# alexj94/future_urban_scene_generation

Hardware: AMD Instinct MI355X
Metric: synthesised vehicle crops/sec @256x256 (higher is better)
Workload: dtype f32 tensors; conv contraction as 3 fp16 MFMA products of scaled (hi, lo) operand splits, f32 accumulate (error vs fp64 <= 1.3x the exact-f32 MFMA kernel's: observed 0.96-1.27x over 12 operand scales x 5 layers; range-guarded; exact-f32 leg in precision_legs)

## Files before the change

### future_urban_scene_generation_amd/_lib.py

```python
from __future__ import annotations

import ctypes as C
import os

_HERE = os.path.dirname(os.path.abspath(__file__))
LIB_PATH = os.environ.get("FUSG_LIB", os.path.join(_HERE, "libfusg.so"))


class FusgUnavailable(RuntimeError):
    pass


class FusgError(RuntimeError):
    pass


class Tensor(C.Structure):
    _fields_ = [("data", C.c_void_p),
                ("n", C.c_int64), ("c", C.c_int64), ("h", C.c_int64), ("w", C.c_int64),
                ("sn", C.c_int64), ("sc", C.c_int64), ("sh", C.c_int64), ("sw", C.c_int64),
                ("dtype", C.c_int32), ("_pad", C.c_int32)]


class ConvDesc(C.Structure):
# ... 5 lines not shown
                ("stride", C.c_int32), ("upsample", C.c_int32), ("pad_mode", C.c_int32), ("pre_op", C.c_int32),
                ("act", C.c_int32), ("store_mode", C.c_int32), ("qh", C.c_int32), ("qw", C.c_int32),
                ("nphase", C.c_int32), ("out_sy", C.c_int32), ("out_sx", C.c_int32),
                ("out_oy", C.c_int32 * 4), ("out_ox", C.c_int32 * 4),
                ("dst_c_off", C.c_int32), ("tile", C.c_int32), ("ksplit", C.c_int32), ("precision", C.c_int32),
                ("wpack_h", C.c_void_p),
                ("kh", C.c_int32), ("kw", C.c_int32), ("dil", C.c_int32), ("pad_h", C.c_int32), ("pad_w", C.c_int32),
                ("wfrag_order", C.c_int32), ("wfrag", C.c_void_p), ("stats_out", C.c_void_p),
                ("tile_list", C.c_void_p), ("tile_count", C.c_int32), ("q_oy", C.c_int32), ("q_ox", C.c_int32),
                ("stats_slots", C.c_int32),
                ("wscale", C.c_void_p), ("status", C.c_void_p), ("wfrag_bf16", C.c_void_p), ("wfrag_f32", C.c_void_p),
                ("splitk_counters", C.c_void_p), ("splitk_counters_len", C.c_int32), ("tap_sparse", C.c_int32)]


class BneckDesc(C.Structure):
    _fields_ = [("x", Tensor), ("res", Tensor), ("dst", Tensor),
                ("pre_scale", C.c_void_p), ("pre_shift", C.c_void_p),
                ("w1frag", C.c_void_p), ("bias1", C.c_void_p), ("wscale1", C.c_void_p),
                ("w2frag", C.c_void_p), ("bias2", C.c_void_p), ("wscale2", C.c_void_p),
                ("w3frag", C.c_void_p), ("bias3", C.c_void_p), ("wscale3", C.c_void_p),
                ("status", C.c_void_p), ("planes", C.c_int32), ("exact_f32", C.c_int32)]


class PackSpec(C.Structure):
    _fields_ = [(n, C.c_int32) for n in ("cout", "cin", "kh", "kw", "c0", "stride", "pad", "dil", "upsample", "cin_pad")]


class PackSizes(C.Structure):
    _fields_ = [("cout_pad", C.c_int32), ("k_pad", C.c_int32), ("c0k", C.c_int32), ("c1k", C.c_int32),
                ("wfrag_order", C.c_int32), ("_pad", C.c_int32), ("wpack_floats", C.c_int64), ("ktab_ints", C.c_int64),
                ("wpack_h_halves", C.c_int64), ("wfrag_halves", C.c_int64)]


F32, U8, I32 = 0, 1, 2
PAD_ZERO, PAD_REFLECT, PAD_REPLICATE = 0, 1, 2
PRE_NONE, PRE_RELU, PRE_ELU, PRE_AFFINE_RELU, PRE_AFFINE = 0, 1, 2, 3, 4
ACT_NONE, ACT_RELU, ACT_TANH, ACT_SIGMOID, ACT_TANH01 = 0, 1, 2, 3, 4
STORE_NORMAL, STORE_D2S, STORE_S2D = 0, 1, 2
PREC_F32, PREC_F16X3, PREC_EMU_BF16, PREC_EMU_BF16X2, PREC_BF16 = 0, 1, 2, 3, 4
MAX_FRAMES = 64
TILE_AUTO, TILE_128x128, TILE_128x64, TILE_128x32, TILE_64x64, TILE_64x128 = 0, 1, 2, 3, 4, 5

_TP = C.POINTER(Tensor)
_SIGS = {
    "fusg_conv2d": (C.c_int, [C.POINTER(ConvDesc), C.c_void_p]),
    "fusg_conv2d_plan": (C.c_int64, [C.POINTER(ConvDesc)]),
    "fusg_conv2d_route": (C.c_int, [C.POINTER(ConvDesc)]),
    "fusg_hg_bottleneck": (C.c_int, [C.POINTER(BneckDesc), C.c_void_p]),
    "fusg_chan_stats": (C.c_int, [_TP, C.c_void_p, C.c_int32, C.c_void_p]),
    "fusg_in_finalize": (C.c_int, [_TP, C.c_void_p, C.c_int32, C.c_float, C.c_void_p, C.c_void_p, C.c_void_p]),
    "fusg_ln_finalize": (C.c_int, [_TP, C.c_void_p, C.c_int32, C.c_float, C.c_void_p, C.c_void_p, C.c_void_p,
                                   C.c_void_p, C.c_void_p]),
    "fusg_in_finalize_slots": (C.c_int, [C.c_void_p, C.c_int32, C.c_int32, C.c_int32, C.c_float, C.c_void_p, C.c_void_p, C.c_void_p]),
    "fusg_ln_finalize_slots": (C.c_int, [C.c_void_p, C.c_int32, C.c_int32, C.c_int32, C.c_float, C.c_void_p, C.c_void_p,
                                         C.c_void_p, C.c_void_p, C.c_void_p]),
    "fusg_affine_act": (C.c_int, [_TP, C.c_void_p, C.c_void_p, C.c_int64, C.c_int32, _TP, _TP, C.c_void_p]),
    "fusg_maxpool2": (C.c_int, [_TP, _TP, C.c_void_p]),
    "fusg_upsample2_add": (C.c_int, [_TP, _TP, _TP, C.c_void_p]),
    "fusg_copy4d": (C.c_int, [_TP, _TP, C.c_int32, C.c_void_p]),
    "fusg_add4d": (C.c_int, [_TP, _TP, _TP, C.c_void_p]),
    "fusg_space_to_depth2": (C.c_int, [_TP, _TP, C.c_void_p]),
    "fusg_depth_to_space2": (C.c_int, [_TP, _TP, C.c_void_p]),
    "fusg_ec_inputs": (C.c_int, [_TP, _TP, _TP, _TP, C.c_int32, C.c_void_p]),
    "fusg_hshift_sum": (C.c_int, [_TP, C.c_void_p, C.c_int32, C.c_int32, C.c_int32, C.c_int32, _TP, C.c_void_p]),
    "fusg_argmax_hw": (C.c_int, [_TP, C.c_void_p, C.c_void_p]),
    "fusg_to_image_u8": (C.c_int, [_TP, _TP, C.c_void_p]),
    "fusg_merge_u8": (C.c_int, [_TP, _TP, _TP, _TP, C.c_void_p]),
    "fusg_warp_perspective_u8": (C.c_int, [_TP, C.c_void_p, _TP, C.c_void_p]),
    "fusg_warp_perspective_indexed_u8": (C.c_int, [_TP, C.c_void_p, C.c_void_p, C.c_int32, _TP, C.c_void_p]),
    "fusg_warp_perspective_frames_u8": (C.c_int, [_TP, C.c_void_p, C.c_void_p, C.c_int32, C.c_int32, _TP, C.c_void_p]),
    "fusg_fill_poly_planes_u8": (C.c_int, [_TP, C.c_void_p, C.c_void_p, C.c_int32, _TP, C.c_void_p]),
# ... 34 lines not shown
    "fusg_plan_destroy": (None, [C.c_void_p]),
    "fusg_plan_begin": (C.c_int, [C.c_void_p]),
    "fusg_plan_end": (C.c_int, [C.c_void_p]),
    "fusg_plan_add_dependency": (C.c_int, [C.c_void_p, C.c_void_p, C.c_void_p]),
    "fusg_plan_add_h2d": (C.c_int, [C.c_void_p, C.c_void_p, C.c_void_p, C.c_int64, C.c_int32, C.c_int64, C.c_void_p]),
    "fusg_plan_next_slot": (C.c_int, [C.c_void_p]),
    "fusg_plan_size": (C.c_int64, [C.c_void_p]),
    "fusg_plan_run": (C.c_int, [C.c_void_p]),
    "fusg_plan_streams": (C.c_int32, [C.c_void_p]),
    "fusg_plan_run_mt": (C.c_int, [C.c_void_p]),
    "fusg_plan_graph_capture": (C.c_int, [C.c_void_p, C.c_void_p, C.c_int32]),
    "fusg_plan_graph_nodes": (C.c_int64, [C.c_void_p]),
    "fusg_plan_graph_slot": (C.c_int, [C.c_void_p]),
    "fusg_plan_graph_launch": (C.c_int, [C.c_void_p, C.c_void_p]),
    "fusg_pack_conv_sizes": (C.c_int, [C.POINTER(PackSpec), C.POINTER(PackSizes)]),
    "fusg_pack_conv_weights": (C.c_int, [C.POINTER(PackSpec)] + [C.c_void_p] * 8),
    "fusg_version": (C.c_int, []),
    "fusg_last_error": (C.c_char_p, []),
    "fusg_last_conv_kernel": (C.c_int, []),
    "fusg_arch": (C.c_char_p, []),
    "fusg_sizeof_tensor": (C.c_int, []),
    "fusg_sizeof_conv_desc": (C.c_int, []),
    "fusg_sizeof_bneck_desc": (C.c_int, []),
    "fusg_prof_enable": (None, [C.c_int]),
    "fusg_prof_reset": (None, []),
    "fusg_prof_read": (C.c_int, [C.c_int, C.POINTER(C.c_double), C.POINTER(C.c_int64), C.POINTER(C.c_double)]),
}
EXPORTS = tuple(_SIGS.keys())

_lib = None


def lib():
    global _lib
    if _lib is None:
        if not os.path.exists(LIB_PATH):
            raise FusgUnavailable(
                f"{LIB_PATH} not found: build it with `python -c 'import __graft_entry__ as g; g.build()'` "
                "(hipcc --offload-arch=gfx950).  There is no CPU fallback.")
        import torch
        try:
            h = C.CDLL(LIB_PATH)
        except OSError as e:
            raise FusgUnavailable(f"cannot load {LIB_PATH}: {e}") from e
        for name, (res, args) in _SIGS.items():
            fn = getattr(h, name)
            fn.restype = res
            fn.argtypes = args
        if (h.fusg_sizeof_tensor() != C.sizeof(Tensor) or h.fusg_sizeof_conv_desc() != C.sizeof(ConvDesc)
                or h.fusg_sizeof_bneck_desc() != C.sizeof(BneckDesc)):
            raise FusgUnavailable("libfusg.so struct layout differs from the ctypes mirror (stale build?)")
        _lib = h
    return _lib


def check(rc: int, what: str = "") -> None:
    if rc != 0:
        msg = lib().fusg_last_error()
        raise FusgError(f"{what}: rc={rc}: {msg.decode() if msg else ''}")
```

### future_urban_scene_generation_amd/csrc/common.h

```cpp
#pragma once
#include <hip/hip_runtime.h>
#include <functional>
#include <memory>
#include <tuple>
#include <utility>
#include <stdint.h>
#include <stdio.h>
#include <string.h>
#include "../../include/fusg.h"

namespace fusg {

void set_error(const char* fmt, ...);
void note_conv_kernel(int kind);

#define FUSG_CHECK(cond, ...)                         \
    do {                                              \
        if (!(cond)) {                                \
            fusg::set_error(__VA_ARGS__);             \
            return FUSG_ERR_INVALID;                  \
        }                                             \
    } while (0)

#define FUSG_LAUNCH_CHECK(what)                                                    \
// ... 32 lines not shown

template <class A> struct SavedArg {
    A a;
    explicit SavedArg(A v) : a(v) {}
    A get() const { return a; }
};
template <> struct SavedArg<const fusg_tensor*> {
    bool has; fusg_tensor t;
    explicit SavedArg(const fusg_tensor* p) : has(p != nullptr), t(p ? *p : fusg_tensor{}) {}
    const fusg_tensor* get() const { return has ? &t : nullptr; }
};
template <> struct SavedArg<const fusg_conv_desc*> {
    bool has; fusg_conv_desc d;
    explicit SavedArg(const fusg_conv_desc* p) : has(p != nullptr), d(p ? *p : fusg_conv_desc{}) {}
    const fusg_conv_desc* get() const { return has ? &d : nullptr; }
};

template <> struct SavedArg<const fusg_bneck_desc*> {
    bool has; fusg_bneck_desc d;
    explicit SavedArg(const fusg_bneck_desc* p) : has(p != nullptr), d(p ? *p : fusg_bneck_desc{}) {}
    const fusg_bneck_desc* get() const { return has ? &d : nullptr; }
};

template <class... A>
int plan_dispatch(int (*impl)(A..., void*), void* stream, A... a) {
    if (plan_recording()) {
        auto saved = std::make_shared<std::tuple<SavedArg<A>...>>(SavedArg<A>(a)...);
        plan_append((hipStream_t)stream, [impl, saved](hipStream_t s) {
            return std::apply([&](const SavedArg<A>&... sv) { return impl(sv.get()..., (void*)s); }, *saved);
        });
    }
    return impl(a..., stream);
}

const float* zero_line();

void prof_begin(int kind, hipStream_t s, double flops);
void prof_end(int kind, hipStream_t s);

}
```

### future_urban_scene_generation_amd/ops.py

```python
from __future__ import annotations

import ctypes as C
from typing import Optional, Tuple

import torch

from . import _lib as L
from .pack import ConvPlan

_DT = {torch.float32: L.F32, torch.uint8: L.U8, torch.int32: L.I32}

import os as _os
import numpy as _np


def _env_set(name: str) -> bool:
    return name in _os.environ


_PREC = {"f32": L.PREC_F32, "f16x3": L.PREC_F16X3,
         "bf16": L.PREC_BF16,
         "emu_bf16": L.PREC_EMU_BF16, "emu_bf16x2": L.PREC_EMU_BF16X2}
_EMU_BITS = {"emu_bf16": 8, "emu_bf16x2": 16}

# ... 444 lines not shown
    d.pre_scale, d.pre_shift = p["pre"][0].data_ptr(), p["pre"][1].data_ptr()
    if RECORDER is not None:
        RECORDER.keep.append(p["pre"])
    for i, key in ((1, "c1"), (2, "c2"), (3, "c3")):
        plan = p[key].to(x.device)
        dev = plan.dev
        if RECORDER is not None:
            RECORDER.keep.append(dev)
        assert dev.get("wfrag") is not None and dev["wfrag_order"] == 0, key
        frag = plan.frag_f32_dev() if f32 else dev["wfrag"]
        assert frag is not None, key
        if RECORDER is not None:
            RECORDER.keep.append(frag)
        setattr(d, "w%dfrag" % i, frag.data_ptr())
        setattr(d, "bias%d" % i, dev["bias"].data_ptr())
        setattr(d, "wscale%d" % i, dev["wscale"].data_ptr())
    d.status = status_word(x.device).data_ptr()
    d.planes = planes
    d.exact_f32 = 1 if f32 else 0
    L.check(L.lib().fusg_hg_bottleneck(C.byref(d), stream_ptr()), "hg_bottleneck")
    return out


def last_conv_kernel() -> int:
    return int(L.lib().fusg_last_conv_kernel())


_BORDER_TILES = {}


def border_tiles(h: int, w: int, device) -> torch.Tensor:
    key = (h, w, str(device))
    t = _BORDER_TILES.get(key)
    if t is None:
        ny, nx = h // 8, w // 16
        idx = [y * nx + x for y in range(ny) for x in range(nx) if y in (0, ny - 1) or x in (0, nx - 1)]
        t = torch.tensor(idx, dtype=torch.int32, device=device)
        _BORDER_TILES[key] = t
    return t


def up2_phases_ok(x: torch.Tensor, precision: Optional[str] = None) -> bool:
    b, c, h, w = x.shape
    return h >= 2 and w >= 2 and _os.environ.get("FUSG_NO_UP2_PHASES") is None


# ... 431 lines not shown
```

### future_urban_scene_generation_amd/vunet/models.py

```python
from __future__ import annotations

import argparse
from typing import List, Optional, Sequence

import torch
import torch.nn as nn

from .. import _lib as L
from .. import ops, pack
from ..nn_base import FusedNet, WNConvP, WNConvTP, entry_point
from .layers import (Activation, DeConv2d, DepthToSpace, DownSample, MyConv2d, NiN, Residual, Sampler, SpaceToDepth,
                     UpSample)


def _res(c_in, c_out, dp, wn):
    return Residual(c_in=c_in, c_out=c_out, activation=Activation("elu"), drop_prob=dp, w_norm=wn)


class AutoRegressiveBlock(nn.Module):
    def __init__(self, drop_prob, w_norm):
        super().__init__()
        self.s2d = SpaceToDepth(2)
        self.d2s = DepthToSpace(2)
        self.residual_init = _res(256, 128, drop_prob, w_norm)
# ... 145 lines not shown
            if name == "shape_decoder_6.conv" and w.shape[0] * w.shape[3] <= 32 and split is None and m.stride == 1:
                P[name] = pack.pack_conv_rowsplit(w, h.bias, pad=m.padding).to(device)
                continue
            P[name] = pack.pack_conv(w, h.bias, c_split=split, stride=m.stride, pad=m.padding).to(device)
        return P

    def _residual(self, name: str, x, skip=None, out=None):
        return ops.conv(self._plans[name + ".layers.2"], x, skip, pre_op=L.PRE_ELU, res0=x, out=out)

    def _nin(self, name: str, x, x1=None, out=None):
        return ops.conv(self._plans[name + ".layers.1"], x, x1, pre_op=L.PRE_ELU, out=out)

    _UP_PLAN = {"subpixel": ".depth4x", "conv2d_t": ".up", "nearest": ".conv"}

    def _upsample(self, name: str, x):
        return ops.conv(self._plans[name + self._UP_PLAN[self.up_mode]], x, store=L.STORE_D2S)

    @staticmethod
    def _subbatch(b: int) -> int:
        import os
        n = int(os.environ.get("FUSG_VU_SUBBATCH", "0"))
        return n if 0 < n < b else 0

    def _shape_encoder_top(self, x, n):
        b, _, h, w = x.shape
        dev = x.device
        sb, sc = ops.nhwc_empty(b, 32, h, w, dev), ops.nhwc_empty(b, 32, h, w, dev)
        ab, ac = ops.nhwc_empty(b, 32, h // 2, w // 2, dev), ops.nhwc_empty(b, 32, h // 2, w // 2, dev)
        a1 = ops.nhwc_empty(b, 32, h // 2, w // 2, dev)
        for lo in range(0, b, n):
            hi = min(b, lo + n)
            t = self._nin("shape_encoder_1.nin", x[lo:hi])
            s0 = self._residual("shape_encoder_1.residual_0", t)
            s1 = self._residual("shape_encoder_1.residual_1", s0)
            self._nin("shape_skip_1_b", s0, out=sb[lo:hi])
            self._nin("shape_skip_1_c", s1, out=sc[lo:hi])
            d = ops.conv(self._plans["shape_encoder_1_a.down.down"], s1)
            a0 = self._residual("shape_encoder_1_a.residual_0", d)
            self._residual("shape_encoder_1_a.residual_1", a0, out=a1[lo:hi])
            self._nin("shape_skip_1_a_b", a0, out=ab[lo:hi])
            self._nin("shape_skip_1_a_c", a1[lo:hi], out=ac[lo:hi])
        return a1, [sb, sc, ab, ac]

    def _shape_decoder_tail(self, x, skips, n):
        b, _, h, w = x.shape
        head = self._plans["shape_decoder_6.conv"]
        out = torch.empty((b, 3, 2 * h, 2 * w), device=x.device, dtype=torch.float32)
        for lo in range(0, b, n):
            hi = min(b, lo + n)
            r = self._residual("shape_decoder_5_a.residual_0", x[lo:hi], skips[0][lo:hi])
            r = self._residual("shape_decoder_5_a.residual_1", r, skips[1][lo:hi])
            u = self._upsample("shape_decoder_5_a.up", r)
            e = self._residual("shape_decoder_6.residual_0", u, skips[2][lo:hi])
            e = self._residual("shape_decoder_6.residual_1", e, skips[3][lo:hi])
            o = ops.conv_rowsplit(head, e, nchw_out=True) if head.rowsplit is not None else ops.conv(head, e, nchw_out=True)
            ops.copy4d(o, out[lo:hi], 0)
        return out

    def set_vehicle_seeds(self, seeds=None):
        if seeds is None:
            self.__dict__.pop("_vehicle_gens", None)
            return
        gens = []
        for sd in seeds:
            g = torch.Generator(device="cpu")
            g.manual_seed(int(sd))
# ... 58 lines not shown
    def _sampler(self, name: str, x, noise, mu_out=None, c_off=0, z_out=None):
        p = self._plans[name + ".conv"]
        if mu_out is None:
            mu = ops.conv(p, x)
        else:
            ops.conv(p, x, out=mu_out, out_c_off=c_off)
            mu = mu_out[:, c_off:c_off + p.cout]
        assert tuple(noise.shape) == tuple(mu.shape), (noise.shape, mu.shape)
        z = ops.add4d(mu, noise, None if z_out is None else z_out[:, c_off:c_off + p.cout])
        return mu, z

    def _init_block(self, name, x):
        x = self._nin(name + ".nin", x)
        s0 = x = self._residual(name + ".residual_0", x)
        s1 = x = self._residual(name + ".residual_1", x)
        return x, [s0, s1]

    def _down_block(self, name, x):
        x = ops.conv(self._plans[name + ".down.down"], x)
        s0 = x = self._residual(name + ".residual_0", x)
        s1 = x = self._residual(name + ".residual_1", x)
        return x, [s0, s1]

    def _up_block(self, name, x, skip_a, skip_b):
        x = self._residual(name + ".residual_0", x, skip_a)
        x = self._residual(name + ".residual_1", x, skip_b)
        return self._upsample(name + ".up", x)

    def _ar_block(self, name, x, skip_a, enc_down_mu, noise):
        x = self._residual(name + ".residual_init", x, skip_a)
        x_ = ops.space_to_depth2(self._residual(name + ".residual_s2d", x))
        g = None
        if enc_down_mu is not None:
            gs = ops.space_to_depth2(ops.as_nhwc(enc_down_mu))
            g = [self._nin(f"{name}.nin_{k}", gs[:, 128 * k:128 * (k + 1)]) for k in range(3)]
        b, _, h, w = x_.shape
        mus = ops.nhwc_empty(b, 512, h, w, x_.device)
        zs = ops.nhwc_empty(b, 512, h, w, x_.device)
        for k in range(4):
            _, z_k = self._sampler(f"{name}.sampler_{k}", x_, noise[k], mus, 128 * k, zs)
            if k < 3:
                cond = g[k] if g is not None else self._nin(f"{name}.nin_{k}", z_k)
                x_ = self._residual(f"{name}.residual_{k}", x_, cond)
        return x, ops.depth_to_space2(mus), ops.depth_to_space2(zs)

    @entry_point
    def forward_enc_up(self, x):
        self._ensure(x)
        x = ops.as_nhwc(x)
        x, _ = self._init_block("app_encoder_1", x)
        names = ["app_encoder_1_a", "app_encoder_1_b"] + (["app_encoder_1_c"] if self.vunet_256 else []) + \
                ["app_encoder_2", "app_encoder_3"]
        for n in names:
            x, _ = self._down_block(n, x)
        skips = [self._nin("app_skip_3_c", x)]
        x, sl = self._down_block("app_encoder_4", x)
        outputs = [sl[-2], x]
        skips.append(self._nin("app_skip_4_c", x))
        return outputs, skips

    @entry_point
    def forward_dec_up(self, x):
        self._ensure(x)
        x = ops.as_nhwc(x)
        skips: List[torch.Tensor] = []
        nsub = self._subbatch(x.shape[0]) if self.vunet_256 else 0
        if nsub:
            x, skips = self._shape_encoder_top(x, nsub)
        else:
            x, sl = self._init_block("shape_encoder_1", x)
            skips += [self._nin("shape_skip_1_b", sl[-2]), self._nin("shape_skip_1_c", sl[-1])]
            if self.vunet_256:
                x, sl = self._down_block("shape_encoder_1_a", x)
                skips += [self._nin("shape_skip_1_a_b", sl[-2]), self._nin("shape_skip_1_a_c", sl[-1])]
        for i in range(2, 7):
            x, sl = self._down_block(f"shape_encoder_{i}", x)
            skips += [self._nin(f"shape_skip_{i}_b", sl[-2]), self._nin(f"shape_skip_{i}_c", sl[-1])]
        return [x], skips

    @entry_point
    def forward_enc_down(self, enc_up_outputs: Sequence[torch.Tensor], skips: Sequence[torch.Tensor]):
        self._ensure(enc_up_outputs[-1])
        P = self._plans
        o1, o2 = ops.as_nhwc(enc_up_outputs[-1]), ops.as_nhwc(enc_up_outputs[-2])
        b, _, h, w = o1.shape
        noise = self._draw_noise([(b, 128, h, w), (b, 128, 2 * h, 2 * w)], o1.device)
        x = ops.conv(P["app_bottleneck"], o1)
        x = self._residual("app_decoder_1_a", x, ops.as_nhwc(skips[-1]))
        mu_0, z_0 = self._sampler("app_decoder_1_b", x, noise[0])
        x_ = ops.conv(P["app_decoder_1_c"], o2, z_0)
        x = self._residual("app_decoder_1_d", x, x_)
        x = self._upsample("app_decoder_1_e", x)
        x = self._residual("app_decoder_2_a", x, None)
        mu_1, z_1 = self._sampler("app_decoder_2_b", x, noise[1])
        return [mu_0, mu_1], [z_0, z_1]

    @entry_point
# ... 55 lines not shown
```

### include/fusg.h

```cpp
#ifndef FUSG_H
#define FUSG_H

#include <stdint.h>

#ifdef __cplusplus
extern "C" {
#endif

#define FUSG_VERSION 118

typedef enum fusg_status {
    FUSG_OK = 0,
    FUSG_ERR_INVALID = -1,
    FUSG_ERR_LAUNCH = -2,
    FUSG_ERR_UNSUPPORTED = -3
} fusg_status;

typedef enum fusg_dtype { FUSG_F32 = 0, FUSG_U8 = 1, FUSG_I32 = 2 } fusg_dtype;

typedef struct fusg_tensor {
    void*   data;
    int64_t n, c, h, w;
    int64_t sn, sc, sh, sw;
    int32_t dtype;
// ... 77 lines not shown
    const void*    wfrag_f32;
    int32_t*       splitk_counters;
    int32_t        splitk_counters_len;
    int32_t        tap_sparse;
} fusg_conv_desc;

int  fusg_conv2d(const fusg_conv_desc* d, void* stream);
int64_t fusg_conv2d_plan(fusg_conv_desc* d);
int  fusg_conv2d_route(const fusg_conv_desc* d);

typedef struct fusg_bneck_desc {
    fusg_tensor x, res, dst;
    const float* pre_scale;
    const float* pre_shift;
    const void*  w1frag; const float* bias1; const float* wscale1;
    const void*  w2frag; const float* bias2; const float* wscale2;
    const void*  w3frag; const float* bias3; const float* wscale3;
    int32_t*     status;
    int32_t      planes;
    int32_t      exact_f32;
} fusg_bneck_desc;
int fusg_hg_bottleneck(const fusg_bneck_desc* d, void* stream);

typedef struct fusg_pack_spec {
    int32_t cout, cin, kh, kw;
    int32_t c0;
    int32_t stride, pad, dil;
    int32_t upsample;
    int32_t cin_pad;
} fusg_pack_spec;
typedef struct fusg_pack_sizes {
    int32_t cout_pad, k_pad, c0k, c1k;
    int32_t wfrag_order;
    int32_t _pad;
    int64_t wpack_floats;
    int64_t ktab_ints;
    int64_t wpack_h_halves;
    int64_t wfrag_halves;
} fusg_pack_sizes;
int fusg_pack_conv_sizes(const fusg_pack_spec* spec, fusg_pack_sizes* sizes);
int fusg_pack_conv_weights(const fusg_pack_spec* spec, const float* weight, const float* bias, float* wpack, int32_t* ktab,
                           float* bias_pad, uint16_t* wpack_h, float* wscale, uint16_t* wfrag);


int fusg_chan_stats(const fusg_tensor* x, float* partial, int32_t nchunk, void* stream);
int fusg_in_finalize(const fusg_tensor* x, const float* partial, int32_t nchunk, float eps,
// ... 127 lines not shown
int        fusg_plan_begin(fusg_plan* p);
int        fusg_plan_end(fusg_plan* p);
int        fusg_plan_add_dependency(fusg_plan* p, void* waiter, void* signaller);
int        fusg_plan_add_h2d(fusg_plan* p, void* dst, const void* src, int64_t bytes, int32_t nslots, int64_t slot_stride, void* stream);
int        fusg_plan_next_slot(fusg_plan* p);
int64_t    fusg_plan_size(const fusg_plan* p);
int        fusg_plan_run(fusg_plan* p);
int32_t    fusg_plan_streams(fusg_plan* p);
int        fusg_plan_run_mt(fusg_plan* p);
int        fusg_plan_graph_capture(fusg_plan* p, void* capture_stream, int32_t slot);
int64_t    fusg_plan_graph_nodes(const fusg_plan* p);
int        fusg_plan_graph_slot(fusg_plan* p);
int        fusg_plan_graph_launch(fusg_plan* p, void* stream);


int         fusg_version(void);
const char* fusg_last_error(void);
enum { FUSG_CONV_GENERIC_F32 = 0, FUSG_CONV_GENERIC_F16X3 = 1, FUSG_CONV_HALO = 2, FUSG_CONV_HALO_S2D = 3,
       FUSG_CONV_TAPUNIT = 4, FUSG_CONV_HALO_BF16 = 5, FUSG_CONV_BNECK = 6 ,
       FUSG_CONV_POINTWISE = 7 ,
       FUSG_CONV_SMALL = 8 ,
       FUSG_CONV_HALO_F32 = 9 ,
       FUSG_CONV_TAPUNIT_F32 = 10 ,
       FUSG_CONV_TAPUNIT_BF16 = 11  };
int         fusg_last_conv_kernel(void);
const char* fusg_arch(void);
int         fusg_sizeof_tensor(void);
int         fusg_sizeof_conv_desc(void);
int         fusg_sizeof_bneck_desc(void);
void fusg_prof_enable(int on);
void fusg_prof_reset(void);
int  fusg_prof_read(int kind, double* total_ms, int64_t* launches, double* flops);

#ifdef __cplusplus
}
#endif
#endif
```

Baseline: 1454.

## Fuse VUNet encoder residual pair and skip NiNs into one kernel

```diff
diff --git a/future_urban_scene_generation_amd/_lib.py b/future_urban_scene_generation_amd/_lib.py
--- a/future_urban_scene_generation_amd/_lib.py
+++ b/future_urban_scene_generation_amd/_lib.py
@@ -51,6 +51,17 @@
                 ("status", C.c_void_p), ("planes", C.c_int32), ("exact_f32", C.c_int32)]
 
 
+class RespairDesc(C.Structure):
+    _fields_ = [("x", Tensor), ("s1", Tensor), ("kb", Tensor), ("kc", Tensor),
+                ("w_in", C.c_void_p), ("bias_in", C.c_void_p),
+                ("wfragA", C.c_void_p), ("biasA", C.c_void_p), ("wscaleA", C.c_void_p),
+                ("wfragB", C.c_void_p), ("biasB", C.c_void_p), ("wscaleB", C.c_void_p),
+                ("wfrag_b", C.c_void_p), ("bias_b", C.c_void_p), ("wscale_b", C.c_void_p),
+                ("wfrag_c", C.c_void_p), ("bias_c", C.c_void_p), ("wscale_c", C.c_void_p),
+                ("status", C.c_void_p), ("channels", C.c_int32), ("entry", C.c_int32),
+                ("cin", C.c_int32), ("kpad_in", C.c_int32), ("tap_order", C.c_int32), ("_pad", C.c_int32)]
+
+
 class PackSpec(C.Structure):
     _fields_ = [(n, C.c_int32) for n in ("cout", "cin", "kh", "kw", "c0", "stride", "pad", "dil", "upsample", "cin_pad")]
 
@@ -76,6 +87,7 @@
     "fusg_conv2d_plan": (C.c_int64, [C.POINTER(ConvDesc)]),
     "fusg_conv2d_route": (C.c_int, [C.POINTER(ConvDesc)]),
     "fusg_hg_bottleneck": (C.c_int, [C.POINTER(BneckDesc), C.c_void_p]),
+    "fusg_vunet_respair": (C.c_int, [C.POINTER(RespairDesc), C.c_void_p]),
     "fusg_chan_stats": (C.c_int, [_TP, C.c_void_p, C.c_int32, C.c_void_p]),
     "fusg_in_finalize": (C.c_int, [_TP, C.c_void_p, C.c_int32, C.c_float, C.c_void_p, C.c_void_p, C.c_void_p]),
     "fusg_ln_finalize": (C.c_int, [_TP, C.c_void_p, C.c_int32, C.c_float, C.c_void_p, C.c_void_p, C.c_void_p,
@@ -156,6 +168,7 @@
     "fusg_sizeof_tensor": (C.c_int, []),
     "fusg_sizeof_conv_desc": (C.c_int, []),
     "fusg_sizeof_bneck_desc": (C.c_int, []),
+    "fusg_sizeof_respair_desc": (C.c_int, []),
     "fusg_prof_enable": (None, [C.c_int]),
     "fusg_prof_reset": (None, []),
     "fusg_prof_read": (C.c_int, [C.c_int, C.POINTER(C.c_double), C.POINTER(C.c_int64), C.POINTER(C.c_double)]),
@@ -182,7 +195,8 @@
             fn.restype = res
             fn.argtypes = args
         if (h.fusg_sizeof_tensor() != C.sizeof(Tensor) or h.fusg_sizeof_conv_desc() != C.sizeof(ConvDesc)
-                or h.fusg_sizeof_bneck_desc() != C.sizeof(BneckDesc)):
+                or h.fusg_sizeof_bneck_desc() != C.sizeof(BneckDesc)
+                or h.fusg_sizeof_respair_desc() != C.sizeof(RespairDesc)):
             raise FusgUnavailable("libfusg.so struct layout differs from the ctypes mirror (stale build?)")
         _lib = h
     return _lib
diff --git a/future_urban_scene_generation_amd/csrc/common.h b/future_urban_scene_generation_amd/csrc/common.h
--- a/future_urban_scene_generation_amd/csrc/common.h
+++ b/future_urban_scene_generation_amd/csrc/common.h
@@ -78,6 +78,12 @@
     const fusg_bneck_desc* get() const { return has ? &d : nullptr; }
 };
 
+template <> struct SavedArg<const fusg_respair_desc*> {
+    bool has; fusg_respair_desc d;
+    explicit SavedArg(const fusg_respair_desc* p) : has(p != nullptr), d(p ? *p : fusg_respair_desc{}) {}
+    const fusg_respair_desc* get() const { return has ? &d : nullptr; }
+};
+
 template <class... A>
 int plan_dispatch(int (*impl)(A..., void*), void* stream, A... a) {
     if (plan_recording()) {
diff --git a/future_urban_scene_generation_amd/csrc/conv_respair.hip b/future_urban_scene_generation_amd/csrc/conv_respair.hip
--- /dev/null
+++ b/future_urban_scene_generation_amd/csrc/conv_respair.hip
@@ -0,0 +1,447 @@
+#include "conv_kernel_h3.h"
+
+namespace fusg {
+
+struct RespairK {
+    const float* x; long xsn, xsh, xsw;
+    float* s1; float* kb; float* kc;
+    long s1n, s1h, s1w, kbn, kbh, kbw, kcn, kch, kcw;
+    const float* w_in; const float* b_in; int cin, kpad_in;
+    const _Float16* wA; const _Float16* wB; const _Float16* wb; const _Float16* wc;
+    const float* bA; const float* bB; const float* bb; const float* bc;
+    const float* sA; const float* sB; const float* sb; const float* sc;
+    const float* zeros;
+    int* status;
+    int B, H, W, tiles_x, tiles_y;
+};
+
+constexpr int RP_XW = 20, RP_XPIX = 12 * 20;
+constexpr int RP_SW = 18, RP_SPIX = 10 * 18;
+constexpr size_t respair_lds(bool entry) { return (size_t)(RP_XPIX + RP_SPIX) * 2 * 32 * sizeof(_Float16) + (entry ? 8 * 32 * sizeof(float) : 0); }
+
+struct RpFrag { h8 f[2][2]; };
+
+__device__ __forceinline__ f32x4 rp_mfma(const h8 a, const h8 b, const f32x4 c) {
+    return __builtin_amdgcn_mfma_f32_16x16x32_f16(a, b, c, 0, 0, 0);
+}
+__device__ __forceinline__ int rp_swz(int hx) { return ((hx >> 2) & 1) << 1; }
+
+__device__ __forceinline__ f32x4 rp_nin(f32x4 xa, const float* pb, bool two, const f32x4 (&w)[8], const f32x4 bias) {
+    f32x4 acc = {0.f, 0.f, 0.f, 0.f};
+#pragma unroll
+    for (int c = 0; c < 4; ++c) xa[c] = elu1(xa[c]);
+    if (two) {
+        f32x4 xb = *(const f32x4*)pb;
+#pragma unroll
+        for (int c = 0; c < 4; ++c) xb[c] = elu1(xb[c]);
+#pragma unroll
+        for (int e = 0; e < 4; ++e)
+#pragma unroll
+            for (int j = 0; j < 4; ++j) acc[j] = fmaf(xb[e], w[4 + e][j], fmaf(xa[e], w[e][j], acc[j]));
+    } else {
+#pragma unroll
+        for (int e = 0; e < 4; ++e)
+#pragma unroll
+            for (int j = 0; j < 4; ++j) acc[j] = fmaf(xa[e], w[e][j], acc[j]);
+    }
+    f32x4 v;
+#pragma unroll
+    for (int j = 0; j < 4; ++j) v[j] = fmaf(acc[j], 1.f, bias[j]);
+    return v;
+}
+
+template <int C, bool ENTRY, bool TAPSPLIT>
+__global__ __launch_bounds__(256, TAPSPLIT ? 1 : 2) void vunet_respair_h3(const RespairK k) {
+    static_assert(C == 32, "one 32-channel chunk per pixel");
+    constexpr int NP = TAPSPLIT ? 4 : 1;
+    extern __shared__ __attribute__((aligned(16))) _Float16 smem_h[];
+    _Float16* Xh = smem_h;
+    _Float16* Xl = Xh + RP_XPIX * 32;
+    _Float16* Sh = Xl + RP_XPIX * 32;
+    _Float16* Sl = Sh + RP_SPIX * 32;
+    float* wl = (float*)(Sl + RP_SPIX * 32);
+
+    const int t = threadIdx.x, lane = t & 63, wave = t >> 6;
+    const int lp = lane & 15, lg = lane >> 4;
+    const int tile = xcd_tile();
+    const int tpi = k.tiles_x * k.tiles_y;
+    const int b = tile / tpi, t2 = tile - b * tpi;
+    const int ty = t2 / k.tiles_x, tx = t2 - ty * k.tiles_x;
+    const int oy0 = ty * 8, ox0 = tx * 16;
+    const float* ximg = k.x + (long)b * k.xsn;
+    float amax = 0.f;
+    const float ninf = -__builtin_inff();
+    const bool two = ENTRY && k.cin > 4;
+
+    constexpr int PF = TAPSPLIT ? 1 : 3, NR = PF + 1;
+    RpFrag wf[NR];
+    auto load_s = [&](int st) __attribute__((always_inline)) {
+        const _Float16* w = (st < 9 ? k.wA : k.wB) + (((st < 9 ? st : st - 9) * 4) * 512 + lane * 8);
+        RpFrag& F = wf[st % NR];
+#pragma unroll
+        for (int ct = 0; ct < 2; ++ct)
+#pragma unroll
+            for (int hl = 0; hl < 2; ++hl) F.f[ct][hl] = *(const h8*)(w + (ct * 2 + hl) * 512);
+    };
+
+    {
+        const int kc = t & 7;
+        f32x4 ra[8];
+        const float* pb[8];
+        unsigned inimg = 0;
+#pragma unroll
+        for (int j = 0; j < 8; ++j) {
+            const int pix = (t + 256 * j) >> 3;
+            const int hy = pix / RP_XW, hx = pix - hy * RP_XW;
+            const int iy = oy0 - 2 + hy, ix = ox0 - 2 + hx;
+            const bool ok = pix < RP_XPIX && (unsigned)iy < (unsigned)k.H && (unsigned)ix < (unsigned)k.W;
+            inimg |= (ok ? 1u : 0u) << j;
+            const float* p = ximg + (long)iy * k.xsh + (long)ix * k.xsw;
+            if constexpr (ENTRY) {
+                ra[j] = *(const f32x4*)(ok ? p : k.zeros);
+                pb[j] = (ok && two) ? p + 4 : k.zeros;
+            } else {
+                ra[j] = *(const f32x4*)(ok ? p + kc * 4 : k.zeros);
+            }
+        }
+        if constexpr (!TAPSPLIT) {
+#pragma unroll
+            for (int st = 0; st < PF; ++st) load_s(st);
+        }
+        f32x4 w[8], bias = {0.f, 0.f, 0.f, 0.f};
+        if constexpr (ENTRY) {
+            const int c = t >> 5, n = t & 31;
+            wl[t] = c < k.cin ? k.w_in[(long)n * k.kpad_in + c] : 0.f;
+            __syncthreads();
+#pragma unroll
+            for (int c2 = 0; c2 < 8; ++c2) w[c2] = *(const f32x4*)(wl + c2 * 32 + kc * 4);
+            bias = *(const f32x4*)(k.b_in + kc * 4);
+        }
+#pragma unroll
+        for (int j = 0; j < 8; ++j) {
+            const int pix = (t + 256 * j) >> 3;
+            const int hy = pix / RP_XW, hx = pix - hy * RP_XW;
+            f32x4 v = ra[j];
+            if constexpr (ENTRY) {
+                v = rp_nin(ra[j], pb[j], two, w, bias);
+                const bool ok = (inimg >> j) & 1u;
+#pragma unroll
+                for (int c = 0; c < 4; ++c) v[c] = ok ? v[c] : 0.f;
+            }
+#pragma unroll
+            for (int c = 0; c < 4; ++c) v[c] = elu1(v[c]);
+            h4 hi, lo;
+            split4<false>(v, ninf, hi, lo, amax);
+            if (pix < RP_XPIX) {
+                const int o = pix * 32 + ((((kc >> 1) ^ rp_swz(hx)) << 3) | ((kc & 1) << 2));
+                *(h4*)(Xh + o) = hi;
+                *(h4*)(Xl + o) = lo;
+            }
+        }
+    }
+
+    int sy[3], sx[3];
+    bool inS[3];
+#pragma unroll
+    for (int i = 0; i < 2; ++i) { sy[i] = 2 * wave + i + 1; sx[i] = lp + 1; inS[i] = true; }
+    {
+        const int q = wave * 16 + lp;
+        inS[2] = q < 52;
+        if (q < 18) { sy[2] = 0; sx[2] = q; }
+        else if (q < 36) { sy[2] = 9; sx[2] = q - 18; }
+        else if (q < 44) { sy[2] = q - 35; sx[2] = 0; }
+        else if (q < 52) { sy[2] = q - 43; sx[2] = 17; }
+        else { sy[2] = 0; sx[2] = 0; }
+    }
+    bool inimg3[3];
+    long goff[3];
+#pragma unroll
+    for (int i = 0; i < 3; ++i) {
+        const int iy = oy0 - 1 + sy[i], ix = ox0 - 1 + sx[i];
+        inimg3[i] = inS[i] && (unsigned)iy < (unsigned)k.H && (unsigned)ix < (unsigned)k.W;
+        goff[i] = (long)iy * k.xsh + (long)ix * k.xsw;
+    }
+    f32x4 resA[3][2], ua[3];
+    const float* pub[3];
+#pragma unroll
+    for (int i = 0; i < 3; ++i) {
+        const float* p = ximg + goff[i];
+        if constexpr (ENTRY) {
+            ua[i] = *(const f32x4*)(inimg3[i] ? p : k.zeros);
+            pub[i] = (inimg3[i] && two) ? p + 4 : k.zeros;
+        } else {
+#pragma unroll
+            for (int ct = 0; ct < 2; ++ct) resA[i][ct] = *(const f32x4*)(inimg3[i] ? p + ct * 16 + lg * 4 : k.zeros);
+        }
+    }
+
+    auto load_w = [&](RpFrag& F, const _Float16* w, int tap) __attribute__((always_inline)) {
+#pragma unroll
+        for (int ct = 0; ct < 2; ++ct)
+#pragma unroll
+            for (int hl = 0; hl < 2; ++hl) F.f[ct][hl] = *(const h8*)(w + ((tap * 2 + ct) * 2 + hl) * 512 + lane * 8);
+    };
+    auto total = [&](const f32x4 (&a)[NP]) __attribute__((always_inline)) {
+        f32x4 s = a[0];
+#pragma unroll
+        for (int q = 1; q < NP; ++q) s += a[q];
+        return s;
+    };
+
+    f32x4 accA[3][2][NP];
+#pragma unroll
+    for (int i = 0; i < 3; ++i)
+#pragma unroll
+        for (int ct = 0; ct < 2; ++ct)
+#pragma unroll
+            for (int q = 0; q < NP; ++q) accA[i][ct][q] = f32x4{0.f, 0.f, 0.f, 0.f};
+    int xbase[3][3];
+#pragma unroll
+    for (int i = 0; i < 3; ++i)
+#pragma unroll
+        for (int kx = 0; kx < 3; ++kx) xbase[i][kx] = (sy[i] * RP_XW + sx[i] + kx) * 32 + ((lg ^ rp_swz(sx[i] + kx)) << 3);
+    if constexpr (TAPSPLIT) load_s(0);
+    __syncthreads();
+#pragma unroll
+    for (int tap = 0; tap < 9; ++tap) {
+        load_s(tap + PF);
+        const RpFrag& F = wf[tap % NR];
+        const int ky = tap / 3, kx = tap - ky * 3;
+        h8 xh[3], xl[3], bs[2];
+#pragma unroll
+        for (int i = 0; i < 3; ++i) {
+            xh[i] = *(const h8*)(Xh + xbase[i][kx] + ky * RP_XW * 32);
+            xl[i] = *(const h8*)(Xl + xbase[i][kx] + ky * RP_XW * 32);
+        }
+#pragma unroll
+        for (int ct = 0; ct < 2; ++ct) bs[ct] = scale_m11(F.f[ct][0]);
+#pragma unroll
+        for (int term = 0; term < 3; ++term)
+#pragma unroll
+            for (int i = 0; i < 3; ++i)
+#pragma unroll
+                for (int ct = 0; ct < 2; ++ct)
+                    accA[i][ct][TAPSPLIT ? (tap & 3) : 0] = rp_mfma(term == 0 ? F.f[ct][0] : term == 1 ? F.f[ct][1] : bs[ct],
+                                                                    term == 2 ? xl[i] : xh[i], accA[i][ct][TAPSPLIT ? (tap & 3) : 0]);
+    }
+
+    f32x4 s0raw[2][2];
+    {
+        f32x4 w[8];
+#pragma unroll
+        for (int ct = 0; ct < 2; ++ct) {
+            const int n0 = ct * 16 + lg * 4;
+            const f32x4 bias = *(const f32x4*)(k.bA + n0), wsc = *(const f32x4*)(k.sA + n0);
+            f32x4 bin = {0.f, 0.f, 0.f, 0.f};
+            if constexpr (ENTRY) {
+#pragma unroll
+                for (int c2 = 0; c2 < 8; ++c2) w[c2] = *(const f32x4*)(wl + c2 * 32 + n0);
+                bin = *(const f32x4*)(k.b_in + n0);
+            }
+#pragma unroll
+            for (int i = 0; i < 3; ++i) {
+                f32x4 r;
+                if constexpr (ENTRY) {
+                    r = rp_nin(ua[i], pub[i], two, w, bin);
+                } else {
+                    r = resA[i][ct];
+                }
+                const f32x4 a = total(accA[i][ct]);
+                f32x4 v;
+#pragma unroll
+                for (int e = 0; e < 4; ++e) { const float y = fmaf(a[e], wsc[e], bias[e]) + r[e]; v[e] = inimg3[i] ? y : 0.f; }
+                if (i < 2) s0raw[i][ct] = v;
+#pragma unroll
+                for (int e = 0; e < 4; ++e) v[e] = elu1(v[e]);
+                h4 hi, lo;
+                split4<false>(v, ninf, hi, lo, amax);
+                if (inS[i]) {
+                    const int o = (sy[i] * RP_SW + sx[i]) * 32 + ((((ct << 1) | (lg >> 1)) ^ rp_swz(sx[i])) << 3) + ((lg & 1) << 2);
+                    *(h4*)(Sh + o) = hi;
+                    *(h4*)(Sl + o) = lo;
+                }
+            }
+        }
+    }
+    __syncthreads();
+    RpFrag wfb, wfc;
+    load_w(wfb, k.wb, 0);
+    load_w(wfc, k.wc, 0);
+
+    f32x4 accB[2][2][NP], accb[2][2], accc[2][2];
+#pragma unroll
+    for (int i = 0; i < 2; ++i)
+#pragma unroll
+        for (int ct = 0; ct < 2; ++ct) {
+#pragma unroll
+            for (int q = 0; q < NP; ++q) accB[i][ct][q] = f32x4{0.f, 0.f, 0.f, 0.f};
+            accb[i][ct] = f32x4{0.f, 0.f, 0.f, 0.f};
+            accc[i][ct] = f32x4{0.f, 0.f, 0.f, 0.f};
+        }
+    int sbase[3];
+#pragma unroll
+    for (int kx = 0; kx < 3; ++kx) sbase[kx] = (2 * wave * RP_SW + lp + kx) * 32 + ((lg ^ rp_swz(lp + kx)) << 3);
+#pragma unroll
+    for (int tap = 0; tap < 9; ++tap) {
+        if (tap + PF < 9) load_s(9 + tap + PF);
+        const RpFrag& F = wf[(9 + tap) % NR];
+        const int ky = tap / 3, kx = tap - ky * 3;
+        h8 xh[2], xl[2], bs[2];
+#pragma unroll
+        for (int i = 0; i < 2; ++i) {
+            xh[i] = *(const h8*)(Sh + sbase[kx] + (ky + i) * RP_SW * 32);
+            xl[i] = *(const h8*)(Sl + sbase[kx] + (ky + i) * RP_SW * 32);
+        }
+#pragma unroll
+        for (int ct = 0; ct < 2; ++ct) bs[ct] = scale_m11(F.f[ct][0]);
+#pragma unroll
+        for (int term = 0; term < 3; ++term)
+#pragma unroll
+            for (int i = 0; i < 2; ++i)
+#pragma unroll
+                for (int ct = 0; ct < 2; ++ct)
+                    accB[i][ct][TAPSPLIT ? (tap & 3) : 0] = rp_mfma(term == 0 ? F.f[ct][0] : term == 1 ? F.f[ct][1] : bs[ct],
+                                                                    term == 2 ? xl[i] : xh[i], accB[i][ct][TAPSPLIT ? (tap & 3) : 0]);
+        if (tap == 4) {
+#pragma unroll
+            for (int ct = 0; ct < 2; ++ct) bs[ct] = scale_m11(wfb.f[ct][0]);
+#pragma unroll
+            for (int term = 0; term < 3; ++term)
+#pragma unroll
+                for (int i = 0; i < 2; ++i)
+#pragma unroll
+                    for (int ct = 0; ct < 2; ++ct)
+                        accb[i][ct] = rp_mfma(term == 0 ? wfb.f[ct][0] : term == 1 ? wfb.f[ct][1] : bs[ct], term == 2 ? xl[i] : xh[i], accb[i][ct]);
+        }
+    }
+
+    _Float16* Th = Xh + wave * 32 * 32;
+    _Float16* Tl = Xl + wave * 32 * 32;
+    const int oxl = ox0 + lp;
+#pragma unroll
+    for (int ct = 0; ct < 2; ++ct) {
+        const int n0 = ct * 16 + lg * 4;
+        const f32x4 biasB = *(const f32x4*)(k.bB + n0), wscB = *(const f32x4*)(k.sB + n0);
+        const f32x4 biasb = *(const f32x4*)(k.bb + n0), wscb = *(const f32x4*)(k.sb + n0);
+#pragma unroll
+        for (int i = 0; i < 2; ++i) {
+            const int oy = oy0 + 2 * wave + i;
+            f32x4 vb, v;
+#pragma unroll
+            for (int e = 0; e < 4; ++e) vb[e] = fmaf(accb[i][ct][e], wscb[e], biasb[e]);
+            *(f32x4*)(k.kb + (long)b * k.kbn + (long)oy * k.kbh + (long)oxl * k.kbw + n0) = vb;
+            const f32x4 a = total(accB[i][ct]);
+#pragma unroll
+            for (int e = 0; e < 4; ++e) v[e] = fmaf(a[e], wscB[e], biasB[e]) + s0raw[i][ct][e];
+            *(f32x4*)(k.s1 + (long)b * k.s1n + (long)oy * k.s1h + (long)oxl * k.s1w + n0) = v;
+#pragma unroll
+            for (int e = 0; e < 4; ++e) v[e] = elu1(v[e]);
+            h4 hi, lo;
+            split4<false>(v, ninf, hi, lo, amax);
+            const int o = (i * 16 + lp) * 32 + ((((ct << 1) | (lg >> 1)) ^ rp_swz(lp)) << 3) + ((lg & 1) << 2);
+            *(h4*)(Th + o) = hi;
+            *(h4*)(Tl + o) = lo;
+        }
+    }
+    __builtin_amdgcn_fence(__ATOMIC_RELEASE, "wavefront");
+    __builtin_amdgcn_wave_barrier();
+    __builtin_amdgcn_fence(__ATOMIC_ACQUIRE, "wavefront");
+    {
+        h8 xh[2], xl[2], bs[2];
+#pragma unroll
+        for (int i = 0; i < 2; ++i) {
+            const int o = (i * 16 + lp) * 32 + ((lg ^ rp_swz(lp)) << 3);
+            xh[i] = *(const h8*)(Th + o);
+            xl[i] = *(const h8*)(Tl + o);
+        }
+#pragma unroll
+        for (int ct = 0; ct < 2; ++ct) bs[ct] = scale_m11(wfc.f[ct][0]);
+#pragma unroll
+        for (int term = 0; term < 3; ++term)
+#pragma unroll
+            for (int i = 0; i < 2; ++i)
+#pragma unroll
+                for (int ct = 0; ct < 2; ++ct)
+                    accc[i][ct] = rp_mfma(term == 0 ? wfc.f[ct][0] : term == 1 ? wfc.f[ct][1] : bs[ct], term == 2 ? xl[i] : xh[i], accc[i][ct]);
+    }
+    if (amax >= F16X3_LIMIT && k.status) *k.status = 1;
+#pragma unroll
+    for (int ct = 0; ct < 2; ++ct) {
+        const int n0 = ct * 16 + lg * 4;
+        const f32x4 bias = *(const f32x4*)(k.bc + n0), wsc = *(const f32x4*)(k.sc + n0);
+#pragma unroll
+        for (int i = 0; i < 2; ++i) {
+            const int oy = oy0 + 2 * wave + i;
+            f32x4 v;
+#pragma unroll
+            for (int e = 0; e < 4; ++e) v[e] = fmaf(accc[i][ct][e], wsc[e], bias[e]);
+            *(f32x4*)(k.kc + (long)b * k.kcn + (long)oy * k.kch + (long)oxl * k.kcw + n0) = v;
+        }
+    }
+}
+
+}
+
+using namespace fusg;
+
+static bool rp_aligned16(const void* p) { return p != nullptr && (((uintptr_t)p) & 15) == 0; }
+
+static int respair_impl(const fusg_respair_desc* d, void* stream) {
+    hipStream_t s = (hipStream_t)stream;
+    FUSG_CHECK(d != nullptr, "vunet_respair: null descriptor");
+    const fusg_tensor& x = d->x;
+    FUSG_CHECK(d->channels == 32, "vunet_respair: channels %d (32 is built)", d->channels);
+    FUSG_CHECK(d->entry == 0 || d->entry == 1, "vunet_respair: entry %d", d->entry);
+    FUSG_CHECK(d->tap_order >= 0 && d->tap_order <= 2, "vunet_respair: tap_order %d", d->tap_order);
+    FUSG_CHECK(is_nhwc(x) && x.n >= 1 && x.h >= 8 && x.w >= 16 && x.h % 8 == 0 && x.w % 16 == 0,
+               "vunet_respair: x must be NHWC-physical f32 with h %% 8 == 0 and w %% 16 == 0 (8 x 16 patches, as the halo kernel)");
+    if (d->entry) {
+        FUSG_CHECK(x.c >= 1 && x.c <= 8 && d->cin >= 4 && d->cin <= 8 && d->cin % 4 == 0 && d->cin <= x.sw && x.c <= d->cin,
+                   "vunet_respair: entry form takes u with at most 8 channels, cin (K-channels of the NiN) 4 or 8 <= its pixel pitch");
+        FUSG_CHECK(rp_aligned16(d->w_in) && rp_aligned16(d->bias_in) && d->kpad_in >= d->cin,
+                   "vunet_respair: the entry NiN's wpack / bias are missing or not 16-byte aligned");
+    } else {
+        FUSG_CHECK(x.c == 32, "vunet_respair: x has %ld channels, not 32", (long)x.c);
+    }
+    const fusg_tensor* outs[3] = {&d->s1, &d->kb, &d->kc};
+    for (const fusg_tensor* o : outs) {
+        FUSG_CHECK(is_nhwc(*o) && same_nhw(x, *o) && o->c == 32, "vunet_respair: s1 / kb / kc must be NHWC-physical f32 [n, 32, h, w] like x");
+        FUSG_CHECK(o->data != x.data, "vunet_respair: an output aliases x (neighbouring patches read x's ring)");
+    }
+    FUSG_CHECK(d->s1.data != d->kb.data && d->s1.data != d->kc.data && d->kb.data != d->kc.data, "vunet_respair: outputs alias each other");
+    const void* ptrs[] = {d->wfragA, d->biasA, d->wscaleA, d->wfragB, d->biasB, d->wscaleB,
+                          d->wfrag_b, d->bias_b, d->wscale_b, d->wfrag_c, d->bias_c, d->wscale_c};
+    for (const void* p : ptrs) FUSG_CHECK(rp_aligned16(p), "vunet_respair: a parameter array is missing or not 16-byte aligned");
+    FUSG_CHECK(d->status != nullptr, "vunet_respair: status word missing");
+    FUSG_CHECK(x.n * x.h * x.w * x.sw < (1L << 40), "vunet_respair: extent");
+    RespairK k;
+    memset(&k, 0, sizeof(k));
+    k.x = (const float*)x.data; k.xsn = x.sn; k.xsh = x.sh; k.xsw = x.sw;
+    k.s1 = (float*)d->s1.data; k.s1n = d->s1.sn; k.s1h = d->s1.sh; k.s1w = d->s1.sw;
+    k.kb = (float*)d->kb.data; k.kbn = d->kb.sn; k.kbh = d->kb.sh; k.kbw = d->kb.sw;
+    k.kc = (float*)d->kc.data; k.kcn = d->kc.sn; k.kch = d->kc.sh; k.kcw = d->kc.sw;
+    k.w_in = d->w_in; k.b_in = d->bias_in; k.cin = d->cin; k.kpad_in = d->kpad_in;
+    k.wA = (const _Float16*)d->wfragA; k.wB = (const _Float16*)d->wfragB; k.wb = (const _Float16*)d->wfrag_b; k.wc = (const _Float16*)d->wfrag_c;
+    k.bA = d->biasA; k.bB = d->biasB; k.bb = d->bias_b; k.bc = d->bias_c;
+    k.sA = d->wscaleA; k.sB = d->wscaleB; k.sb = d->wscale_b; k.sc = d->wscale_c;
+    k.status = d->status;
+    k.zeros = zero_line();
+    if (!k.zeros) { set_error("vunet_respair: cannot allocate the zero line"); return FUSG_ERR_LAUNCH; }
+    k.B = (int)x.n; k.H = (int)x.h; k.W = (int)x.w;
+    k.tiles_x = k.W / 16; k.tiles_y = k.H / 8;
+    const long wgs = (long)k.B * k.tiles_x * k.tiles_y;
+    FUSG_CHECK(wgs < (1L << 31), "vunet_respair: grid");
+    const bool split = d->tap_order == 0 ? (!env_switches().no_ksplit && wgs <= 1024) : d->tap_order == 2;
+    const void* fn = d->entry ? (split ? (const void*)vunet_respair_h3<32, true, true> : (const void*)vunet_respair_h3<32, true, false>)
+                              : (split ? (const void*)vunet_respair_h3<32, false, true> : (const void*)vunet_respair_h3<32, false, false>);
+    const size_t lds = respair_lds(d->entry != 0);
+    const double M = (double)x.n * x.h * x.w;
+    prof_begin(0, s, 2.0 * M * 32.0 * ((d->entry ? (double)d->kpad_in : 0.0) + 2.0 * 9.0 * 32.0 + 2.0 * 32.0));
+    const hipError_t e = launch_kernel(fn, dim3((unsigned)wgs), lds, (int)lds, k, s);
+    prof_end(0, s);
+    if (e != hipSuccess) { set_error("vunet_respair launch: %s", hipGetErrorString(e)); return FUSG_ERR_LAUNCH; }
+    note_conv_kernel(FUSG_CONV_RESPAIR);
+    return FUSG_OK;
+}
+extern "C" int fusg_vunet_respair(const fusg_respair_desc* d, void* stream) { return fusg::plan_dispatch(respair_impl, stream, d); }
+extern "C" int fusg_sizeof_respair_desc(void) { return (int)sizeof(fusg_respair_desc); }
diff --git a/future_urban_scene_generation_amd/ops.py b/future_urban_scene_generation_amd/ops.py
--- a/future_urban_scene_generation_amd/ops.py
+++ b/future_urban_scene_generation_amd/ops.py
@@ -490,6 +490,73 @@
     return out
 
 
+VU_RESPAIR = not _env_set("FUSG_NO_RESPAIR")
+
+
+def respair_ok(res_a: ConvPlan, res_b: ConvPlan, nin_b: ConvPlan, nin_c: ConvPlan, x: torch.Tensor,
+               nin_in: Optional[ConvPlan] = None, precision: Optional[str] = None) -> bool:
+    prec = precision or PRECISION
+    if not VU_RESPAIR or prec != "f16x3" or not is_nhwc(x):
+        return False
+    for p in (res_a, res_b):
+        if not (p.cout == 32 and p.cout_pad == 32 and p.c0k == 32 and p.c1k == 0 and p.kh == 3 and p.kw == 3 and p.pad == 1
+                and p.pad_w < 0 and p.stride == 1 and p.dil == 1 and p.upsample == 0 and p.nphase == 1 and p.pad_mode == L.PAD_ZERO):
+            return False
+    for p in (nin_b, nin_c):
+        if not (p.cout == 32 and p.cout_pad == 32 and p.c0k == 32 and p.c1k == 0 and p.kh == 1 and p.kw == 1 and p.pad == 0
+                and p.stride == 1 and p.nphase == 1):
+            return False
+    b, c, h, w = x.shape
+    if nin_in is not None:
+        if not (nin_in.cout == 32 and nin_in.cout_pad == 32 and nin_in.c0k in (4, 8) and nin_in.c1k == 0 and nin_in.kh == 1
+                and nin_in.kw == 1 and nin_in.pad == 0 and nin_in.stride == 1 and nin_in.nphase == 1 and c == nin_in.c_split[0]):
+            return False
+    elif c != 32:
+        return False
+    key = (id(res_b), id(nin_b), id(nin_c), id(nin_in), b, c, h, w, x.stride(3), str(x.device),
+           _env_set("FUSG_NO_SMALL"), _env_set("FUSG_NO_POINTWISE"), _env_set("FUSG_SMALL_KSPLIT"))
+    memo = res_a.__dict__.setdefault("_respair_routes", {})
+    if key not in memo:
+        t32 = x if nin_in is None else nhwc_empty(b, 32, h, w, x.device)
+        asks = [(res_a, t32, t32, 2), (res_b, t32, t32, 2), (nin_b, t32, None, 2), (nin_c, t32, None, 2)]
+        if nin_in is not None:
+            asks.append((nin_in, x, None, 7))
+        ok = True
+        for plan, src, res, family in asks:
+            d, _ = _conv_desc(plan, src, pre_op=L.PRE_ELU, res0=res, out=t32, precision=prec)
+            L.lib().fusg_conv2d_plan(C.byref(d))
+            ok = ok and L.lib().fusg_conv2d_route(C.byref(d)) == family
+        memo[key] = ok
+    return memo[key]
+
+
+def respair(res_a: ConvPlan, res_b: ConvPlan, nin_b: ConvPlan, nin_c: ConvPlan, x: torch.Tensor,
+            nin_in: Optional[ConvPlan] = None, tap_order: int = 0):
+    b, _, h, w = x.shape
+    s1, kb, kc = (nhwc_empty(b, 32, h, w, x.device) for _ in range(3))
+    d = L.RespairDesc()
+    d.x, d.s1, d.kb, d.kc = desc(x), desc(s1), desc(kb), desc(kc)
+    for key, plan in (("A", res_a), ("B", res_b), ("_b", nin_b), ("_c", nin_c)):
+        dev = plan.to(x.device).dev
+        if RECORDER is not None:
+            RECORDER.keep.append(dev)
+        assert dev.get("wfrag") is not None and dev["wfrag_order"] == 0, key
+        setattr(d, "wfrag" + key, dev["wfrag"].data_ptr())
+        setattr(d, "bias" + key, dev["bias"].data_ptr())
+        setattr(d, "wscale" + key, dev["wscale"].data_ptr())
+    if nin_in is not None:
+        dev = nin_in.to(x.device).dev
+        if RECORDER is not None:
+            RECORDER.keep.append(dev)
+        d.w_in, d.bias_in = dev["wpack"].data_ptr(), dev["bias"].data_ptr()
+        d.entry, d.cin, d.kpad_in = 1, nin_in.c0k, nin_in.k_pad
+    d.status = status_word(x.device).data_ptr()
+    d.channels = 32
+    d.tap_order = int(tap_order)
+    L.check(L.lib().fusg_vunet_respair(C.byref(d), stream_ptr()), "vunet_respair")
+    return s1, kb, kc
+
+
 def last_conv_kernel() -> int:
     return int(L.lib().fusg_last_conv_kernel())
 
diff --git a/future_urban_scene_generation_amd/vunet/models.py b/future_urban_scene_generation_amd/vunet/models.py
--- a/future_urban_scene_generation_amd/vunet/models.py
+++ b/future_urban_scene_generation_amd/vunet/models.py
@@ -191,26 +191,6 @@
         n = int(os.environ.get("FUSG_VU_SUBBATCH", "0"))
         return n if 0 < n < b else 0
 
-    def _shape_encoder_top(self, x, n):
-        b, _, h, w = x.shape
-        dev = x.device
-        sb, sc = ops.nhwc_empty(b, 32, h, w, dev), ops.nhwc_empty(b, 32, h, w, dev)
-        ab, ac = ops.nhwc_empty(b, 32, h // 2, w // 2, dev), ops.nhwc_empty(b, 32, h // 2, w // 2, dev)
-        a1 = ops.nhwc_empty(b, 32, h // 2, w // 2, dev)
-        for lo in range(0, b, n):
-            hi = min(b, lo + n)
-            t = self._nin("shape_encoder_1.nin", x[lo:hi])
-            s0 = self._residual("shape_encoder_1.residual_0", t)
-            s1 = self._residual("shape_encoder_1.residual_1", s0)
-            self._nin("shape_skip_1_b", s0, out=sb[lo:hi])
-            self._nin("shape_skip_1_c", s1, out=sc[lo:hi])
-            d = ops.conv(self._plans["shape_encoder_1_a.down.down"], s1)
-            a0 = self._residual("shape_encoder_1_a.residual_0", d)
-            self._residual("shape_encoder_1_a.residual_1", a0, out=a1[lo:hi])
-            self._nin("shape_skip_1_a_b", a0, out=ab[lo:hi])
-            self._nin("shape_skip_1_a_c", a1[lo:hi], out=ac[lo:hi])
-        return a1, [sb, sc, ab, ac]
-
     def _shape_decoder_tail(self, x, skips, n):
         b, _, h, w = x.shape
         head = self._plans["shape_decoder_6.conv"]
@@ -315,6 +295,30 @@
         s1 = x = self._residual(name + ".residual_1", x)
         return x, [s0, s1]
 
+    def _respair(self, name, skip, x, nin_in=None):
+        P = self._plans
+        plans = (P[name + ".residual_0.layers.2"], P[name + ".residual_1.layers.2"], P[skip + "_b.layers.1"], P[skip + "_c.layers.1"])
+        if not ops.respair_ok(*plans, x, nin_in=nin_in):
+            return None
+        s1, kb, kc = ops.respair(*plans, x, nin_in=nin_in)
+        return s1, [kb, kc]
+
+    def _init_block_skips(self, name, skip, x):
+        fused = self._respair(name, skip, x, nin_in=self._plans[name + ".nin.layers.1"])
+        if fused is not None:
+            return fused
+        x, sl = self._init_block(name, x)
+        return x, [self._nin(skip + "_b", sl[-2]), self._nin(skip + "_c", sl[-1])]
+
+    def _down_block_skips(self, name, skip, x):
+        d = ops.conv(self._plans[name + ".down.down"], x)
+        fused = self._respair(name, skip, d)
+        if fused is not None:
+            return fused
+        s0 = self._residual(name + ".residual_0", d)
+        s1 = self._residual(name + ".residual_1", s0)
+        return s1, [self._nin(skip + "_b", s0), self._nin(skip + "_c", s1)]
+
     def _up_block(self, name, x, skip_a, skip_b):
         x = self._residual(name + ".residual_0", x, skip_a)
         x = self._residual(name + ".residual_1", x, skip_b)
@@ -357,15 +361,11 @@
         self._ensure(x)
         x = ops.as_nhwc(x)
         skips: List[torch.Tensor] = []
-        nsub = self._subbatch(x.shape[0]) if self.vunet_256 else 0
-        if nsub:
-            x, skips = self._shape_encoder_top(x, nsub)
-        else:
-            x, sl = self._init_block("shape_encoder_1", x)
-            skips += [self._nin("shape_skip_1_b", sl[-2]), self._nin("shape_skip_1_c", sl[-1])]
-            if self.vunet_256:
-                x, sl = self._down_block("shape_encoder_1_a", x)
-                skips += [self._nin("shape_skip_1_a_b", sl[-2]), self._nin("shape_skip_1_a_c", sl[-1])]
+        x, sk = self._init_block_skips("shape_encoder_1", "shape_skip_1", x)
+        skips += sk
+        if self.vunet_256:
+            x, sk = self._down_block_skips("shape_encoder_1_a", "shape_skip_1_a", x)
+            skips += sk
         for i in range(2, 7):
             x, sl = self._down_block(f"shape_encoder_{i}", x)
             skips += [self._nin(f"shape_skip_{i}_b", sl[-2]), self._nin(f"shape_skip_{i}_c", sl[-1])]
diff --git a/include/fusg.h b/include/fusg.h
--- a/include/fusg.h
+++ b/include/fusg.h
@@ -123,6 +123,22 @@
 } fusg_bneck_desc;
 int fusg_hg_bottleneck(const fusg_bneck_desc* d, void* stream);
 
+typedef struct fusg_respair_desc {
+    fusg_tensor x, s1, kb, kc;
+    const float* w_in; const float* bias_in;
+    const void*  wfragA;  const float* biasA;  const float* wscaleA;
+    const void*  wfragB;  const float* biasB;  const float* wscaleB;
+    const void*  wfrag_b; const float* bias_b; const float* wscale_b;
+    const void*  wfrag_c; const float* bias_c; const float* wscale_c;
+    int32_t*     status;
+    int32_t      channels;
+    int32_t      entry;
+    int32_t      cin, kpad_in;
+    int32_t      tap_order;
+    int32_t      _pad;
+} fusg_respair_desc;
+int fusg_vunet_respair(const fusg_respair_desc* d, void* stream);
+
 typedef struct fusg_pack_spec {
     int32_t cout, cin, kh, kw;
     int32_t c0;
@@ -296,12 +312,14 @@
        FUSG_CONV_SMALL = 8 ,
        FUSG_CONV_HALO_F32 = 9 ,
        FUSG_CONV_TAPUNIT_F32 = 10 ,
-       FUSG_CONV_TAPUNIT_BF16 = 11  };
+       FUSG_CONV_TAPUNIT_BF16 = 11 ,
+       FUSG_CONV_RESPAIR = 12  };
 int         fusg_last_conv_kernel(void);
 const char* fusg_arch(void);
 int         fusg_sizeof_tensor(void);
 int         fusg_sizeof_conv_desc(void);
 int         fusg_sizeof_bneck_desc(void);
+int         fusg_sizeof_respair_desc(void);
 void fusg_prof_enable(int on);
 void fusg_prof_reset(void);
 int  fusg_prof_read(int kind, double* total_ms, int64_t* launches, double* flops);
```

Result: faster. 1484 (median of 6 runs) (+2.1%).
